# Picsart-AI-Research/MI-GAN

Hardware: AMD Instinct MI355X
Metric: images/sec migan-512 generator fwd (higher is better)
Workload: dtype f32; 1 GPU; migan-512 generator forward, batch=32 per GPU, 512x512, fp32 (BASELINE configs[2]); global_batch=32, resolution=512, parallelism=batch-shard x1, activation_storage=f32, streams=2, weights=static (migan_assume_static_weights: 1x1 operand planes prepared once)

## Files before the change

mi-gan_amd/csrc/migan_pipe.hpp:

```cpp
#pragma once

namespace migan {

constexpr int kPipeBWaves = 8;
constexpr int pipe_threads(int na) { return (na + kPipeBWaves) * 64; }

template <int MODE, int NT, int CIN, bool FROMRGB, int R>
struct PipeLds {
  static constexpr int NKC = CIN / 32;
  static constexpr int IN_SLOT = 1536 * 16;
  static constexpr int A_BUF = 2 * 128 * 64;
  static constexpr int B_CHUNK = 2 * NT * 64;
  static constexpr bool WRES = NKC * B_CHUNK <= 32 * 1024;
  static constexpr int NBUF_B = WRES ? NKC : 2;
  static constexpr int OFF_IN = 0;
  static constexpr int OFF_A = OFF_IN + R * IN_SLOT;
  static constexpr int OFF_B = OFF_A + 2 * A_BUF;
  static constexpr int OFF_W = OFF_B + NBUF_B * B_CHUNK;
  static constexpr bool TAPS_RES = NKC <= 8;
  static constexpr int OFF_F = OFF_W + (TAPS_RES ? NKC : 2) * 1280;
  static constexpr int F_SZ = FROMRGB ? NKC * 3 * 32 * 32 : 0;
  static constexpr int OFF_RGB = OFF_F + F_SZ;
  static constexpr int RGB_BUF = 192 * 32;
  static constexpr int OFF_T = OFF_RGB + (FROMRGB ? 2 * RGB_BUF : 0);
// ... 421 lines not shown
              const int hp = p.HO >> 1, wp = p.WO >> 1;
              const int row = lane / 10, col = lane - row * 10;
              const int yy = ((wtc.y * p.sy - p.off) >> 1) - 1 + row, xx = ((wtc.x * p.sx - p.off) >> 1) - 1 + col;
              const bool ok = lane < 60 && yy >= 0 && yy < hp && xx >= 0 && xx < wp;
              const unsigned voff = ok ? (unsigned)(yy * wp + xx) * 4u : 0xfffff000u;
              float* pw = reinterpret_cast<float*>(lds + L::OFF_PW + (wk & 1) * L::PW_SZ);
#pragma unroll
              for (int ch = 0; ch < 3; ++ch) MIGAN_LDS_DMA4(pbuf, voff, (unsigned)((wtc.b * 3 + ch) * hp * wp) * 4u, pw + ch * 64);
            }
            ++wk;
            if (wk < T) tile_next(wtc);
          }
          wstep = wstep + 1 == NKC ? 0 : wstep + 1;
        }
      };
      for (int g = 0; g < G; ++g) {
        if constexpr (!WRES) { if (g >= 1) issue_b(); }
        issue_prev_window();
        issue_in();
        if constexpr (!TAPS_RES) { if (g + 2 < G) load_taps((dc + 1) % NKC); }
        PPROF_MARK(0);
        if (g + 1 < G) depthwise(dslot, dc, (g + 1) & 1);
        PPROF_MARK(1);
        if constexpr (!TAPS_RES) { if (g + 2 < G) store_taps(g & 1); }
        dslot = dslot + 1 == R ? 0 : dslot + 1;
        dc = dc + 1 == NKC ? 0 : dc + 1;
        if (R == 3 && g + 3 < G) MIGAN_WAIT_VMCNT(DNI); else MIGAN_WAIT_VMCNT(0);
        PPROF_MARK(2);
        MIGAN_BARRIER_LDS();
        PPROF_MARK(3);
      }
    }
    if constexpr (TORGB) MIGAN_BARRIER_LDS();
    if constexpr (MODE == MODE_UP) {
#pragma unroll
      for (int i = 0; i < 2 * (NT / 64) - 1; ++i) MIGAN_BARRIER_LDS();
    }
    PPROF_END(AT);
    return;
  }

  const int tb = tid - AT, wb = wave_u - NA;
  const int rb = wb & 3, cbk = wb >> 2;
  const int l31 = lane & 31, half = lane >> 5;
  (void)tb;
  f16v acc[NTIW], accp[NTIW];
#pragma unroll
  for (int j = 0; j < NTIW; ++j)
#pragma unroll
    for (int r = 0; r < 16; ++r) { acc[j][r] = 0.0f; accp[j][r] = 0.0f; }

  auto mfma_chunk = [&](int abuf, int bbuf, bool first) {
    const char* ab = lds + L::OFF_A + abuf * L::A_BUF;
    const char* bb = lds + L::OFF_B + bbuf * L::B_CHUNK;
#pragma unroll
    for (int ks = 0; ks < KC / 16; ++ks) {
      f4 av[NPL], bv[NTIW][NPL];
      {
        const int row = rb * 32 + l31;
        const char* q = ab + row * PB + (((2 * ks + half) ^ ((row >> 2) & (NSLOT - 1))) << 4);
#pragma unroll
        for (int pl = 0; pl < NPL; ++pl) av[pl] = ld4(reinterpret_cast<const float*>(q + pl * MT * PB));
      }
#pragma unroll
      for (int j = 0; j < NTIW; ++j) {
        const int row = cbk * (NT / 2) + j * 32 + l31;
        const char* q = bb + row * PB + (((2 * ks + half) ^ ((row >> 2) & (NSLOT - 1))) << 4);
#pragma unroll
        for (int pl = 0; pl < NPL; ++pl) bv[j][pl] = ld4(reinterpret_cast<const float*>(q + pl * NT * PB));
      }
#pragma unroll
      for (int j = 0; j < NTIW; ++j) {
        if (first && ks == 0) acc[j] = f16v{0.f, 0.f, 0.f, 0.f, 0.f, 0.f, 0.f, 0.f, 0.f, 0.f, 0.f, 0.f, 0.f, 0.f, 0.f, 0.f};
        acc[j] = MIGAN_MFMA_F16_32X32X16(av[1], bv[j][0], acc[j]);
      }
#pragma unroll
      for (int j = 0; j < NTIW; ++j) acc[j] = MIGAN_MFMA_F16_32X32X16(av[0], bv[j][1], acc[j]);
#pragma unroll
      for (int j = 0; j < NTIW; ++j) acc[j] = MIGAN_MFMA_F16_32X32X16(av[0], bv[j][0], acc[j]);
    }
  };

  const float acc_scale = reinterpret_cast<const float*>(p.wsplit)[-4];
  const bool has_noise = p.noise != nullptr;
  const float ns = has_noise ? p.noise_strength[0] : 0.0f;
  const size_t img_out_bytes = (size_t)p.HO * p.WO * p.CO * 4;

  int ck = 0, cn0 = 0, cb0 = 0, cgy0 = 0, cgx0 = 0, pn0 = 0, pb0 = 0, pgy0 = 0, pgx0 = 0;
  int ppar = 0;
  TileCur ctc = tile0;
  tile_coords(ctc, cn0, cb0, cgy0, cgx0);
  auto hand_over = [&]() {
#pragma unroll
    for (int j = (MODE == MODE_NORMAL ? 1 : 0); j < NTIW; ++j) accp[j] = acc[j];
    pn0 = cn0; pb0 = cb0; pgy0 = cgy0; pgx0 = cgx0; ppar = ck & 1;
    if (++ck < T) { tile_next(ctc); tile_coords(ctc, cn0, cb0, cgy0, cgx0); }
  };

  BuildCursor bcur;
  if constexpr (FROMRGB) build_begin(bcur);
  auto build_step = [&](BuildCursor& bc) {
    build_units(bc, NA == 8 && wb >= 3 ? -1 : wb, 8);
    build_advance(bc);
  };
  MIGAN_BARRIER_LDS();
  if constexpr (FROMRGB) {
    build_step(bcur);
    build_step(bcur);
  }
  MIGAN_BARRIER_LDS();
  MIGAN_BARRIER_LDS();

  if constexpr (MODE == MODE_NORMAL) {
    float* const t_s = reinterpret_cast<float*>(lds + L::OFF_T) + wb * (32 * 32);
    const int q4 = lane & 7, prow = lane >> 3;
    int twr[4];
    {
      const int u = (l31 >> 2) ^ (2 * half);
#pragma unroll
      for (int v = 0; v < 4; ++v) twr[v] = (4 * half) * 32 + ((u ^ ((v & 1) + 4 * (v >> 1))) << 2) + (l31 & 3);
    }
    const int trd0 = prow * 32 + ((q4 ^ (prow >> 1)) << 2), trd1 = prow * 32 + ((q4 ^ (prow >> 1) ^ 4) << 2);
    float nz[4] = {0.f, 0.f, 0.f, 0.f};
    float nzn[4] = {0.f, 0.f, 0.f, 0.f};
    float rs[4][3];
    unsigned pix0 = 0;
    f4 tw[NTIW][3];
    float tbias[3] = {0.f, 0.f, 0.f};
    if constexpr (TORGB) {
#pragma unroll
      for (int ch = 0; ch < 3; ++ch) tbias[ch] = p.trgb_b[ch];
#pragma unroll
      for (int j = 0; j < NTIW; ++j)
#pragma unroll
        for (int ch = 0; ch < 3; ++ch) tw[j][ch] = ld4(p.trgb_w + ch * p.CO + cbk * (NT / 2) + j * 32 + q4 * 4);
    }
    float* const part_s = reinterpret_cast<float*>(lds + L::OFF_P) + rb * (32 * 4);
    u4v u8c = {0u, 0u, 0u, 0u}, u8n = {0u, 0u, 0u, 0u};
    auto request_next = [&]() {
      if (has_noise) {
        const unsigned px = (unsigned)((cgy0 + 2 * rb) * p.WO + cgx0 + prow) * 4u;
#pragma unroll
        for (int q = 0; q < 4; ++q) nzn[q] = *at_bytes(p.noise + ((q >> 1) * p.WO + (q & 1) * 8), px);
      }
      if constexpr (TORGB) {
        if (p.u8_out && cbk == 0 && q4 < 4)
          u8n = fetch_pixel_bytes(p.u8_img, p.u8_mask, (size_t)cb0 * p.HO * p.WO + (size_t)(cgy0 + 2 * rb + (q4 >> 1)) * p.WO + cgx0 + (q4 & 1) * 8 + prow);
      }
    };
    auto begin_tile_epilogue = [&]() {
      pix0 = (unsigned)((pgy0 + 2 * rb) * p.WO + pgx0 + prow);
#pragma unroll
      for (int q = 0; q < 4; ++q) nz[q] = nzn[q];
      if constexpr (TORGB) {
        u8c = u8n;
#pragma unroll
        for (int q = 0; q < 4; ++q) rs[q][0] = rs[q][1] = rs[q][2] = 0.0f;
      }
    };
    auto stage_block = [&](const f16v& a) {
      MIGAN_WAVE_SYNC();
#pragma unroll
      for (int r = 0; r < 16; ++r) t_s[twr[((r >> 1) & 1) + 2 * ((r >> 2) & 1)] + ((r & 3) + 8 * (r >> 2)) * 32] = a[r];
      MIGAN_WAVE_SYNC();
    };
    f4 tv[4];
    auto fetch_block = [&]() {
#pragma unroll
      for (int q = 0; q < 4; ++q) tv[q] = ld4(t_s + ((q & 1) ? trd1 : trd0) + q * 8 * 32);
    };
    const bool store_y = !TORGB || p.y != nullptr;
    auto finish_block = [&](int j) {
      char* yb = reinterpret_cast<char*>(p.y) + (size_t)pb0 * img_out_bytes;
      if constexpr (TORGB) {
        const unsigned col = (unsigned)(pn0 + cbk * (NT / 2) + j * 32 + q4 * 4);
        f4 v[4];
#pragma unroll
        for (int q = 0; q < 4; ++q) v[q] = act4(tv[q] * acc_scale + MIGAN_FMUL_RN(nz[q], ns));
        if (store_y) {
#pragma unroll
          for (int q = 0; q < 4; ++q) {
            const unsigned pix = pix0 + (unsigned)((q >> 1) * p.WO + (q & 1) * 8);
            Io<0>::st(yb, (pix * (unsigned)p.CO + col) * 4u, v[q]);
          }
        }
#pragma unroll
        for (int q = 0; q < 4; ++q) {
          float r0, r1, r2;
          torgb_partial(v[q], tw[j][0], tw[j][1], tw[j][2], r0, r1, r2);
          rs[q][0] += r0; rs[q][1] += r1; rs[q][2] += r2;
        }
      } else {
#pragma unroll
        for (int q = 0; q < 4; ++q) {
          f4 v = tv[q] * acc_scale + MIGAN_FMUL_RN(nz[q], ns);
          v = act4(v);
          const unsigned pix = pix0 + (unsigned)((q >> 1) * p.WO + (q & 1) * 8);
          Io<0>::st(yb, (pix * (unsigned)p.CO + (unsigned)(pn0 + cbk * (NT / 2) + j * 32 + q4 * 4)) * 4u, v);
        }
      }
    };
    float mine[3] = {0.f, 0.f, 0.f};
    auto rgb_partials = [&]() {
#pragma unroll
      for (int q = 0; q < 4; ++q) {
        const float s0 = MIGAN_SUM8(rs[q][0]), s1 = MIGAN_SUM8(rs[q][1]), s2 = MIGAN_SUM8(rs[q][2]);
        if (q4 == q) { mine[0] = s0; mine[1] = s1; mine[2] = s2; }
      }
      if (cbk == 1 && q4 < 4) st4(part_s + (8 * q4 + prow) * 4, f4{mine[0], mine[1], mine[2], 0.0f});
    };
    auto rgb_finish = [&]() {
      if (cbk == 0 && q4 < 4) {
        const f4 other = ld4(part_s + (8 * q4 + prow) * 4);
        const size_t plane = (size_t)p.HO * p.WO;
        const int oy = pgy0 + 2 * rb + (q4 >> 1), ox = pgx0 + (q4 & 1) * 8 + prow;
        float o3[3] = {mine[0] + other.x, mine[1] + other.y, mine[2] + other.z};
        MIGAN_OPAQUE_F(o3[0]); MIGAN_OPAQUE_F(o3[1]); MIGAN_OPAQUE_F(o3[2]);
        o3[0] += tbias[0]; MIGAN_OPAQUE_F(o3[0]);
        o3[1] += tbias[1]; MIGAN_OPAQUE_F(o3[1]);
        o3[2] += tbias[2]; MIGAN_OPAQUE_F(o3[2]);
        if (p.img_prev) {
          const int y0 = (oy & 1) ? (oy >> 1) : (oy >> 1) - 1, x0 = (ox & 1) ? (ox >> 1) : (ox >> 1) - 1;
          const float wy0 = (oy & 1) ? 0.75f : 0.25f, wx0 = (ox & 1) ? 0.75f : 0.25f;
          const float* pw = reinterpret_cast<const float*>(lds + L::OFF_PW + ppar * L::PW_SZ) + (y0 - (pgy0 >> 1) + 1) * 10 + (x0 - (pgx0 >> 1) + 1);
#pragma unroll
          for (int ch = 0; ch < 3; ++ch) {
            const float r0 = wx0 * pw[ch * 64] + (1.0f - wx0) * pw[ch * 64 + 1];
            const float r1 = wx0 * pw[ch * 64 + 10] + (1.0f - wx0) * pw[ch * 64 + 11];
            o3[ch] = (wy0 * r0 + (1.0f - wy0) * r1) + o3[ch];
          }
        }
        if (p.u8_out) {
          compose_pixel_bytes(u8c, p.u8_out, (size_t)pb0 * plane + (size_t)oy * p.WO + ox, o3[0], o3[1], o3[2]);
        } else {
          const unsigned po = (unsigned)(oy * p.WO + ox) * 4u;
#pragma unroll
          for (int ch = 0; ch < 3; ++ch) *at_bytes(p.img_out + ((size_t)pb0 * 3 + ch) * plane, po) = o3[ch];
        }
      }
    };
#pragma unroll
    for (int c = 0; c < NKC; ++c) {
      mfma_chunk(c & 1, WRES ? c : (c & 1), c == 0);
      if (c == NKC - 1) {
        request_next();
        stage_block(acc[0]);
        hand_over();
      }
      if constexpr (FROMRGB) build_step(bcur);
      MIGAN_BARRIER_LDS();
    }
    for (int t = 1; t < T; ++t) {
#pragma unroll
      for (int c = 0; c < NKC; ++c) {
        PPROF_MARK(7);
        if (c < NTIW) fetch_block();
        mfma_chunk(c & 1, WRES ? c : (c & 1), c == 0);
        PPROF_MARK(4);
        if (c == NKC - 1) request_next();
        PPROF_MARK(12);
        if (c == 0) begin_tile_epilogue();
        PPROF_MARK(5);
        if (c < NTIW) {
          finish_block(c);
          if (c + 1 < NTIW) stage_block(accp[c + 1 < NTIW ? c + 1 : 0]);
        }
        PPROF_MARK(9);
        if constexpr (TORGB) {
          if (c == NTIW - 1) rgb_partials();
          PPROF_MARK(10);
          if (c == NTIW) rgb_finish();
          PPROF_MARK(11);
        }
        if (c == NKC - 1) {
          stage_block(acc[0]);
          hand_over();
        }
        PPROF_MARK(7);
        if constexpr (FROMRGB) build_step(bcur);
        PPROF_MARK(13);
        MIGAN_BARRIER_LDS();
        PPROF_MARK(6);
      }
    }
    begin_tile_epilogue();
#pragma unroll
    for (int j = 0; j < NTIW; ++j) {
      fetch_block();
      finish_block(j);
      if (j + 1 < NTIW) stage_block(accp[j + 1 < NTIW ? j + 1 : 0]);
    }
    if constexpr (TORGB) {
      rgb_partials();
      MIGAN_BARRIER_LDS();
      rgb_finish();
    }
  } else {
    constexpr int GS = 64 + 4, QN = 16, LG_QN = 4, NH = NT / 64;
    static_assert(NT == 64 || NT == 128, "FIR-up tiles: 64 or 128 output channels");
    constexpr int SP = NKC / NH;
    static_assert(NKC % NH == 0 && SP >= 2, "too few K steps to hide the FIR epilogue under");
    constexpr int BT = kPipeBWaves * 64;
    constexpr int STEP = BT >> LG_QN;
    constexpr int ITEMS = MT * QN / BT;
    float* const g_s = reinterpret_cast<float*>(lds + L::OFF_T);
    auto acc_to_lds = [&](int h) {
      if (NH == 2 && cbk != h) return;
#pragma unroll
      for (int j = 0; j < NTIW; ++j)
#pragma unroll
        for (int r = 0; r < 16; ++r) {
          const int row = rb * 32 + (r & 3) + 8 * (r >> 2) + 4 * half;
          const int ly = pgy0 + (row >> lgGW), lx = pgx0 + (row & (GW - 1));
          float v = accp[j][r];
          if (ly < 0 || ly >= p.H || lx < 0 || lx >= p.W) v = 0.0f;
          g_s[row * GS + (NH == 2 ? j * 32 : cbk * 32) + l31] = v;
        }
    };
    const int c4 = tb & (QN - 1), m0 = tb >> LG_QN;
    struct ItemIo {
      f4 sk[2][2];
      float nzv[2][2];
    };
    auto item_geo = [&](int k, int h, int& m, unsigned& lpix, unsigned& loff) -> bool {
      m = m0 + k * STEP;
      const int gy = m >> lgGW, gx = m & (GW - 1);
      if (gy < 1 || gy > GH - 2 || gx < 1 || gx > GW - 2) return false;
      const int ly = pgy0 + gy, lx = pgx0 + gx;
      if (ly >= p.H || lx >= p.W) return false;
      lpix = (unsigned)((2 * ly) * p.WO + 2 * lx);
      loff = (lpix * (unsigned)p.CO + (unsigned)(pn0 + h * 64 + c4 * 4)) * 4u;
      return true;
    };
    auto item_load = [&](int k, int h, ItemIo& io) {
      int m;
      unsigned lpix, loff;
      if (!item_geo(k, h, m, lpix, loff)) return;
      const char* sb = p.skip ? reinterpret_cast<const char*>(p.skip) + (size_t)pb0 * img_out_bytes : nullptr;
#pragma unroll
      for (int a = 0; a < 2; ++a)
#pragma unroll
        for (int bb = 0; bb < 2; ++bb) {
          const unsigned dp = (unsigned)(a * p.WO + bb);
          io.nzv[a][bb] = has_noise ? p.noise[lpix + dp] : 0.0f;
          io.sk[a][bb] = sb ? Io<0>::ld_once(sb, loff + dp * (unsigned)p.CO * 4u) : f4{0.f, 0.f, 0.f, 0.f};
        }
    };
    auto item_finish = [&](int k, int h, const ItemIo& io) {
      int m;
      unsigned lpix, loff;
      if (!item_geo(k, h, m, lpix, loff)) return;
      char* yb = reinterpret_cast<char*>(p.y) + (size_t)pb0 * img_out_bytes;
      f4 e[3], o[3];
#pragma unroll
      for (int dy = 0; dy < 3; ++dy) {
        const float* gp = g_s + (m + (dy - 1) * GW) * GS + c4 * 4;
        const f4 l = ld4(gp - GS), ctr = ld4(gp), rgt = ld4(gp + GS);
        e[dy] = 0.25f * l + 0.75f * ctr;
        o[dy] = 0.75f * ctr + 0.25f * rgt;
      }
      f4 out[2][2];
      out[0][0] = 0.25f * e[0] + 0.75f * e[1];
      out[0][1] = 0.25f * o[0] + 0.75f * o[1];
      out[1][0] = 0.75f * e[1] + 0.25f * e[2];
      out[1][1] = 0.75f * o[1] + 0.25f * o[2];
#pragma unroll
      for (int a = 0; a < 2; ++a)
#pragma unroll
        for (int bb = 0; bb < 2; ++bb) {
          f4 v = out[a][bb] * acc_scale + MIGAN_FMUL_RN(io.nzv[a][bb], ns);
          v = act4(v);
          v += io.sk[a][bb];
          Io<0>::st(yb, loff + (unsigned)(a * p.WO + bb) * (unsigned)p.CO * 4u, v);
        }
    };
    constexpr int SL = SP - 1;
    auto slice_of = [](int k) { return k * SL / ITEMS; };
    ItemIo io[2];
#pragma unroll
    for (int c = 0; c < NKC; ++c) {
      mfma_chunk(c & 1, WRES ? c : (c & 1), c == 0);
      if (c == NKC - 1) hand_over();
      MIGAN_BARRIER_LDS();
    }
    for (int t = 1; t < T; ++t) {
#pragma unroll
      for (int c = 0; c < NKC; ++c) {
        constexpr int dummy = 0; (void)dummy;
        const int h = c / SP, cs = c % SP;
        if (cs >= 1) {
#pragma unroll
          for (int k = 0; k < ITEMS; ++k)
            if (slice_of(k) == cs - 1 && (k == 0 || slice_of(k - 1) != cs - 1)) item_load(k, h, io[k & 1]);
        }
        PPROF_MARK(7);
        mfma_chunk(c & 1, WRES ? c : (c & 1), c == 0);
        PPROF_MARK(4);
        if (cs == 0) {
          acc_to_lds(h);
        } else {
#pragma unroll
          for (int k = 0; k < ITEMS; ++k)
            if (slice_of(k) == cs - 1) {
              if (k + 1 < ITEMS && slice_of(k + 1) == cs - 1) item_load(k + 1, h, io[(k + 1) & 1]);
              item_finish(k, h, io[k & 1]);
            }
        }
        if (c == NKC - 1) hand_over();
        PPROF_MARK(5);
        MIGAN_BARRIER_LDS();
        PPROF_MARK(6);
      }
    }
#pragma unroll
    for (int h = 0; h < NH; ++h) {
      if (h > 0) MIGAN_BARRIER_LDS();
      acc_to_lds(h);
      MIGAN_BARRIER_LDS();
      item_load(0, h, io[0]);
#pragma unroll
      for (int k = 0; k < ITEMS; ++k) {
        if (k + 1 < ITEMS) item_load(k + 1, h, io[(k + 1) & 1]);
        item_finish(k, h, io[k & 1]);
      }
    }
  }
  PPROF_MARK(5);
  PPROF_END(AT);
}

template <int NT, int CIN, int R>
struct DownLds {
  static constexpr int KC = 16, NKC = CIN / KC;
  static constexpr int IN_UNITS = 12 * 36 * 4;
  static constexpr int A_BUF = 2 * 64 * 32;
  static constexpr int B_CHUNK = 2 * NT * 32;
  static constexpr bool WRES = NKC * B_CHUNK <= 32 * 1024;
  static constexpr int NBUF_B = WRES ? NKC : 2;
  static constexpr int DWP = 17;
  static constexpr int D_SZ = 10 * 2 * DWP * KC * 4;
  static constexpr int IN_SLOT = IN_UNITS * 16;
  static constexpr int OFF_D = R * IN_SLOT;
  static constexpr int OFF_A = OFF_D + D_SZ;
  static constexpr int OFF_B = OFF_A + 2 * A_BUF;
  static constexpr int OFF_W = OFF_B + NBUF_B * B_CHUNK;
  static constexpr int OFF_T = OFF_W + NKC * 640;
  template <int NB> static constexpr int total() { return OFF_T + NB * 32 * 32 * 4; }
};

template <int NT, int CIN, int R, int NA, int NB>
MIGAN_GLOBAL void MIGAN_LAUNCH_BOUNDS((NA + NB) * 64, (NA + NB) / 4) sepconv_pipedown_kernel(const SepArgs p) {
  typedef DownLds<NT, CIN, R> L;
  constexpr int AT = NA * 64, KC = 16, QC = 4, LG_QC = 2, NKC = L::NKC, MT = 64, GH = 4, GW = 16, lgGW = 4;
  constexpr int IGH = 12, IGW = 36, NPIXW = IGH * IGW, NITEMS = NPIXW * QC, DH = 10, DW = 34, DH2 = 5, DWP = L::DWP;
  constexpr int DNI = (NITEMS + AT - 1) / AT;
  constexpr bool WRES = L::WRES;
  constexpr int DNB = (4 * NT + AT - 1) / AT;
  static_assert(NB == 4 || NB == 8, "2 row blocks x 2 or 4 column groups");
  constexpr int NTIW = NT * 2 / (32 * NB);
  constexpr bool DEFER = NTIW <= 2;
  static_assert(NTIW <= NKC, "one epilogue block per K step");
  static_assert(NT == 128 || NT == 256, "one workgroup owns 128 or 256 output channels");
  static_assert(R == 2, "two-slot ring");
  static_assert(L::template total<NB>() <= 160 * 1024, "LDS budget");
  MIGAN_DYN_SMEM(smem);
  char* const lds = reinterpret_cast<char*>(smem);
  constexpr int IN_SLOT = L::IN_SLOT, OFF_D = L::OFF_D, OFF_A = L::OFF_A, OFF_B = L::OFF_B, OFF_W = L::OFF_W, OFF_T = L::OFF_T;

  const int tid = threadIdx.x;
  const int lane = tid & 63;
  const int wave_u = MIGAN_UNIFORM(tid >> 6);
  const bool groupA = tid < AT;
  const int HO = p.H >> 1, WO = p.W >> 1;

  const int ntiles = p.tiles_x * p.tiles_y * p.nchunks * p.B;
  const int xcd = (int)blockIdx.x & 7;
  const int tq = ntiles >> 3, tr = ntiles & 7;
  const int tcnt = tq + (xcd < tr ? 1 : 0);
  const int tbase = xcd < tr ? xcd * (tq + 1) : tr * (tq + 1) + (xcd - tr) * tq;
  const int tstep = ((int)gridDim.x + 7 - xcd) >> 3;
  const int tl0 = (int)blockIdx.x >> 3;
  const int T = tl0 < tcnt ? (tcnt - tl0 + tstep - 1) / tstep : 0;
  if (T == 0) return;
  const int G = T * NKC;
  PPROF_BEGIN();
  struct TileCur {
    int n, x, y, b;
  };
  const int st_n = tstep % p.nchunks, st_r1 = tstep / p.nchunks;
  const int st_x = st_r1 % p.tiles_x, st_r2 = st_r1 / p.tiles_x;
  const int st_y = st_r2 % p.tiles_y, st_b = st_r2 / p.tiles_y;
  TileCur tile0;
  {
    int t = tbase + tl0;
    tile0.n = t % p.nchunks; t /= p.nchunks;
    tile0.x = t % p.tiles_x; t /= p.tiles_x;
    tile0.y = t % p.tiles_y;
    tile0.b = t / p.tiles_y;
  }
  auto tile_next = [&](TileCur& c) {
    int carry = 0;
    c.n += st_n;
    if (c.n >= p.nchunks) { c.n -= p.nchunks; carry = 1; }
    c.x += st_x + carry; carry = 0;
    if (c.x >= p.tiles_x) { c.x -= p.tiles_x; carry = 1; }
    c.y += st_y + carry; carry = 0;
    if (c.y >= p.tiles_y) { c.y -= p.tiles_y; carry = 1; }
    c.b += st_b + carry;
  };

  if (groupA) {
    MIGAN_SETPRIO(2);
    const int lt = tid;
    float* const w_s = reinterpret_cast<float*>(lds + OFF_W);
    float* const d_s = reinterpret_cast<float*>(lds + OFF_D);
    for (int i = lt; i < CIN * 9 / 4; i += AT) {
      const f4 v = ld4(p.wdw + i * 4);
#pragma unroll
      for (int e = 0; e < 4; ++e) {
        const int f = i * 4 + e, ch = f / 9, tap = f - ch * 9;
        w_s[(ch >> 4) * 160 + tap * 16 + (ch & 15)] = v[e];
      }
    }
    for (int i = lt; i < CIN / 4; i += AT) st4(w_s + ((i * 4) >> 4) * 160 + 144 + ((i * 4) & 15), ld4(p.bdw + i * 4));

    const MIGAN_BUF wbuf = MIGAN_MAKE_BUF(p.wsplit, (unsigned)(2 * p.CO * CIN) * 2u);
    const bool bshort = MIGAN_UNIFORM((DNB - 1) * AT + wave_u * 64) >= 4 * NT;
    unsigned dboff[DNB];
#pragma unroll
    for (int j = 0; j < DNB; ++j) {
      const int u = lt + j * AT;
      const int plane = u / (2 * NT), rem = u % (2 * NT);
      dboff[j] = (unsigned)(plane * p.CO * CIN + (rem >> 1) * 32 + (rem & 1) * 8) * 2u;
    }
    auto dma_b = [&](int n0_, int chunk, int buf) {
      float* bb = reinterpret_cast<float*>(lds + OFF_B + buf * L::B_CHUNK);
      const unsigned soff = (unsigned)((chunk >> 1) * 32 * p.CO + n0_ * 32 + (chunk & 1) * 16) * 2u;
#pragma unroll
      for (int j = 0; j < DNB; ++j)
        if (j + 1 < DNB || !bshort) MIGAN_LDS_DMA16(wbuf, dboff[j], soff, bb + (j * AT + wave_u * 64) * 4);
    };
    const bool dshort = MIGAN_UNIFORM((DNI - 1) * AT + wave_u * 64) >= NITEMS;
    unsigned dgoff[DNI], drel[DNI], tile_soff = 0;
#pragma unroll
    for (int j = 0; j < DNI; ++j) {
      const int i = lt + j * AT;
      drel[j] = 0xfffff000u;
      if (i < NITEMS) {
        const int c4 = i & (QC - 1), pix = i >> LG_QC;
        drel[j] = (unsigned)(((pix / IGW) * p.W + (pix % IGW)) * CIN + c4 * 4) * 4u;
      }
    }
    auto make_dgoff = [&](int gy0_, int gx0_) {
      const int iy0 = 2 * gy0_ - 2, ix0 = 2 * gx0_ - 2;
      if (iy0 >= 0 && iy0 + IGH <= p.H && ix0 >= 0 && ix0 + IGW <= p.W) {
#pragma unroll
        for (int j = 0; j < DNI; ++j) dgoff[j] = drel[j];
        tile_soff = (unsigned)((iy0 * p.W + ix0) * CIN) * 4u;
        return;
      }
      tile_soff = 0;
#pragma unroll
      for (int j = 0; j < DNI; ++j) {
        const int i = lt + j * AT;
        unsigned g = 0xfffff000u;
        if (i < NITEMS) {
          const int c4 = i & (QC - 1), pix = i >> LG_QC;
          const int yy = iy0 + pix / IGW, xx = ix0 + pix % IGW;
          if (yy >= 0 && yy < p.H && xx >= 0 && xx < p.W) g = (unsigned)((yy * p.W + xx) * CIN + c4 * 4) * 4u;
        }
        dgoff[j] = g;
      }
    };
    const unsigned img_bytes = (unsigned)(p.H * p.W * CIN) * 4u;
    auto dma_in = [&](int b0_, int chunk, int slot) {
      float* in_s = reinterpret_cast<float*>(lds + slot * IN_SLOT);
      const MIGAN_BUF xbuf = MIGAN_MAKE_BUF(reinterpret_cast<const char*>(p.x) + (size_t)b0_ * img_bytes, img_bytes);
#pragma unroll
      for (int j = 0; j < DNI; ++j)
        if (j + 1 < DNI || !dshort) MIGAN_LDS_DMA16(xbuf, dgoff[j], tile_soff + (unsigned)(chunk * KC) * 4u, in_s + (j * AT + wave_u * 64) * 4);
    };
    auto stage1 = [&](int slot, int chunk, int gy0_, int gx0_) {
      const float* in_s = reinterpret_cast<const float*>(lds + slot * IN_SLOT);
      const float* wc = w_s + chunk * 160;
      const int c4 = lt & (QC - 1);
      f4 w[9];
#pragma unroll
      for (int tap = 0; tap < 9; ++tap) w[tap] = ld4(wc + tap * KC + c4 * 4);
      const f4 bias = ld4(wc + KC * 9 + c4 * 4);
      const int yim0 = 2 * gy0_ - 1, xim0 = 2 * gx0_ - 1;
      for (int it = lt; it < DH2 * DW * QC; it += AT) {
        const int r = it >> LG_QC;
        const int dx = r % DW, dy0 = 2 * (r / DW);
        const float* ip = in_s + (dy0 * IGW + dx) * KC + c4 * 4;
        f4 win[4][3];
#pragma unroll
        for (int rr = 0; rr < 4; ++rr) {
          win[rr][0] = ld4(ip); win[rr][1] = ld4(ip + KC); win[rr][2] = ld4(ip + 2 * KC);
          ip += IGW * KC;
        }
        const int xim = xim0 + dx;
        const bool colin = xim >= 0 && xim < p.W;
        float* dp = d_s + ((dy0 * 2 + (dx & 1)) * DWP + (dx >> 1)) * KC + c4 * 4;
        f4 dv[2];
#pragma unroll
        for (int o = 0; o < 2; ++o) {
          f4 sacc = bias;
#pragma unroll
          for (int ky = 0; ky < 3; ++ky)
#pragma unroll
            for (int kx = 0; kx < 3; ++kx) sacc += w[ky * 3 + kx] * win[o + ky][kx];
          const int yim = yim0 + dy0 + o;
          dv[o] = f4{0.f, 0.f, 0.f, 0.f};
          if (colin && yim >= 0 && yim < p.H) dv[o] = act4(sacc);
        }
        st4(dp, 0.125f * dv[0] + 0.375f * dv[1]);
        st4(dp + 2 * DWP * KC, 0.375f * dv[0] + 0.125f * dv[1]);
      }
    };
    auto stage2 = [&](int abuf) {
      char* a_b = lds + OFF_A + abuf * L::A_BUF;
      for (int it = lt; it < MT * QC; it += AT) {
        const int c4 = it & (QC - 1), m = it >> LG_QC;
        const int ox = m & (GW - 1), oy = m >> lgGW;
        const float* dp = d_s + ((2 * oy) * 2 * DWP + ox) * KC + c4 * 4;
        f4 a = {0.f, 0.f, 0.f, 0.f};
#pragma unroll
        for (int kx = 0; kx < 4; ++kx) {
          const float fx = (kx == 0 || kx == 3) ? 0.125f : 0.375f;
          const float* q = dp + ((kx & 1) * DWP + (kx >> 1)) * KC;
          a += fx * (ld4(q) + ld4(q + 3 * 2 * DWP * KC));
        }
        u2v h1, h2;
        split2_f16(a * kF16AScale, h1, h2);
        char* d = a_b + m * 32 + c4 * 8;
        *reinterpret_cast<u2v*>(d) = h1;
        *reinterpret_cast<u2v*>(d + MT * 32) = h2;
      }
    };

    int is = 0, ic = 0, ik = 0, ib0 = 0, in0 = 0, igy0 = 0, igx0 = 0;
    TileCur itc = tile0;
    auto icoords = [&]() { in0 = itc.n * NT; ib0 = itc.b; igy0 = itc.y * GH; igx0 = itc.x * GW; };
    icoords();
    make_dgoff(igy0, igx0);
    auto issue = [&]() {
      if (is < G) {
        dma_in(ib0, ic, is & 1);
        ++is;
        if (++ic == NKC) {
          ic = 0;
          if (++ik < T) { tile_next(itc); icoords(); make_dgoff(igy0, igx0); }
        }
      }
    };
    int bs = 0, bc = 0, bk = 0, bn0 = in0;
    TileCur btc = tile0;
    auto issue_b = [&]() -> bool {
      if (bs >= G) return false;
      dma_b(bn0, bc, bs & 1);
      ++bs;
      if (++bc == NKC) {
        bc = 0;
        if (++bk < T) { tile_next(btc); bn0 = btc.n * NT; }
      }
      return true;
    };
    int dk = 0, dc = 0, dgy0 = igy0, dgx0 = igx0;
    TileCur dtc = tile0;
    auto dadvance = [&]() {
      if (++dc == NKC) {
        dc = 0;
        if (++dk < T) { tile_next(dtc); dgy0 = dtc.y * GH; dgx0 = dtc.x * GW; }
      }
    };
    if constexpr (WRES) {
#pragma unroll
      for (int c = 0; c < NKC; ++c) dma_b(in0, c, c);
    } else {
      issue_b();
      issue_b();
    }
    issue();
    issue();
    if (dshort) MIGAN_WAIT_VMCNT(DNI - 1); else MIGAN_WAIT_VMCNT(DNI);
    MIGAN_BARRIER_LDS();
    stage1(0, 0, dgy0, dgx0);
    MIGAN_BARRIER_LDS();
    stage2(0);
    dadvance();
    MIGAN_WAIT_VMCNT(0);
    MIGAN_BARRIER_LDS();
    for (int g = 0; g < G; ++g) {
      issue();
      PPROF_MARK(0);
      if (g + 1 < G) stage1((g + 1) & 1, dc, dgy0, dgx0);
      PPROF_MARK(1);
      MIGAN_BARRIER_LDS();
      PPROF_MARK(3);
      if (g + 1 < G) { stage2((g + 1) & 1); dadvance(); }
      PPROF_MARK(14);
      bool newer = false;
      if constexpr (!WRES) newer = issue_b();
      if (newer && !bshort) MIGAN_WAIT_VMCNT(DNB); else if (newer && DNB > 1) MIGAN_WAIT_VMCNT(DNB > 1 ? DNB - 1 : 0); else MIGAN_WAIT_VMCNT(0);
      PPROF_MARK(2);
      MIGAN_BARRIER_LDS();
      PPROF_MARK(3);
    }
    PPROF_END(AT);
    return;
  }

  const int wb = wave_u - NA;
  const int rb = wb & 1, cb = wb >> 1;
  const int l31 = lane & 31, half = lane >> 5;
  f16v acc[NTIW], accp[DEFER ? NTIW : 1];
#pragma unroll
  for (int j = 0; j < NTIW; ++j)
#pragma unroll
    for (int r = 0; r < 16; ++r) { acc[j][r] = 0.0f; if (DEFER) accp[j][r] = 0.0f; }
  auto mfma_chunk = [&](int abuf, int bbuf, bool first) {
    const char* ab = lds + OFF_A + abuf * L::A_BUF + (rb * 32 + l31) * 32 + half * 16;
    const char* bb = lds + OFF_B + bbuf * L::B_CHUNK + half * 16;
    const f4 a_hi = ld4(reinterpret_cast<const float*>(ab)), a_lo = ld4(reinterpret_cast<const float*>(ab + MT * 32));
    f4 b_hi[NTIW], b_lo[NTIW];
#pragma unroll
    for (int j = 0; j < NTIW; ++j) {
      const char* q = bb + ((cb * NTIW + j) * 32 + l31) * 32;
// ... 125 lines not shown
```

Measured before the change: 3662 images/sec.

## Compact FIR-up epilogue item map to interior pixels and hand-schedule item loads

The FIR-up epilogue used to map work items over the whole halo tile and discard border ones with branches. It now maps items only over interior pixels, clamping coordinates so every lane does useful work, and replaces the general slice schedule with a fixed three-item schedule. Noise and skip loads become branch-free masked loads from a dummy pointer, and the first item's loads are issued during hand-over to hide latency. The static_asserts tie the code to a single 64-column phase with exactly three items, so other tile shapes will no longer compile.

```diff
diff --git a/mi-gan_amd/csrc/migan_pipe.hpp b/mi-gan_amd/csrc/migan_pipe.hpp
--- a/mi-gan_amd/csrc/migan_pipe.hpp
+++ b/mi-gan_amd/csrc/migan_pipe.hpp
@@ -747,7 +747,12 @@
     static_assert(NKC % NH == 0 && SP >= 2, "too few K steps to hide the FIR epilogue under");
     constexpr int BT = kPipeBWaves * 64;
     constexpr int STEP = BT >> LG_QN;
-    constexpr int ITEMS = MT * QN / BT;
+    constexpr int IH = GH - 2, IW = GW - 2;
+    constexpr int NIT = IH * IW * QN;
+    constexpr int FULL = NIT / BT, ITEMS = (NIT + BT - 1) / BT;
+    constexpr int RWAVES = (NIT - FULL * BT) / 64;
+    static_assert((NIT - FULL * BT) % 64 == 0, "the remainder of the item map must be whole waves");
+    static_assert(NH == 1 && FULL == 2 && ITEMS == 3 && SP - 1 == ITEMS, "item schedule: one 64-column phase, items 0 and 1 for all, item 2 for RWAVES waves");
     float* const g_s = reinterpret_cast<float*>(lds + L::OFF_T);
     auto acc_to_lds = [&](int h) {
       if (NH == 2 && cbk != h) return;
@@ -763,38 +768,41 @@
         }
     };
     const int c4 = tb & (QN - 1), m0 = tb >> LG_QN;
+    const bool third = wb < RWAVES;
+    const bool has_skip = p.skip != nullptr;
     struct ItemIo {
       f4 sk[2][2];
       float nzv[2][2];
     };
-    auto item_geo = [&](int k, int h, int& m, unsigned& lpix, unsigned& loff) -> bool {
-      m = m0 + k * STEP;
-      const int gy = m >> lgGW, gx = m & (GW - 1);
-      if (gy < 1 || gy > GH - 2 || gx < 1 || gx > GW - 2) return false;
-      const int ly = pgy0 + gy, lx = pgx0 + gx;
-      if (ly >= p.H || lx >= p.W) return false;
-      lpix = (unsigned)((2 * ly) * p.WO + 2 * lx);
+    auto item_geo = [&](int k, int h, int& m, unsigned& lpix, unsigned& loff) {
+      const int q = m0 + k * STEP;
+      const int ty = 1 + q / IW, tx = 1 + q % IW, ylast = p.H - 1 - pgy0, xlast = p.W - 1 - pgx0;
+      const int gy = ty < ylast ? ty : ylast, gx = tx < xlast ? tx : xlast;
+      m = (gy << lgGW) + gx;
+      lpix = (unsigned)((2 * (pgy0 + gy)) * p.WO + 2 * (pgx0 + gx));
       loff = (lpix * (unsigned)p.CO + (unsigned)(pn0 + h * 64 + c4 * 4)) * 4u;
-      return true;
-    };
-    auto item_load = [&](int k, int h, ItemIo& io) {
+    };
+    auto item_load = [&](int k, int h, ItemIo& io, bool live) {
       int m;
       unsigned lpix, loff;
-      if (!item_geo(k, h, m, lpix, loff)) return;
-      const char* sb = p.skip ? reinterpret_cast<const char*>(p.skip) + (size_t)pb0 * img_out_bytes : nullptr;
+      item_geo(k, h, m, lpix, loff);
+      const bool ln = has_noise && live, ls = has_skip && live;
+      const float* nb = ln ? p.noise : reinterpret_cast<const float*>(p.wsplit);
+      const char* sb = ls ? reinterpret_cast<const char*>(p.skip) + (size_t)pb0 * img_out_bytes : reinterpret_cast<const char*>(p.wsplit);
+      const unsigned nmask = ln ? ~0u : 0u, smask = ls ? ~0u : 0u;
 #pragma unroll
       for (int a = 0; a < 2; ++a)
 #pragma unroll
         for (int bb = 0; bb < 2; ++bb) {
           const unsigned dp = (unsigned)(a * p.WO + bb);
-          io.nzv[a][bb] = has_noise ? p.noise[lpix + dp] : 0.0f;
-          io.sk[a][bb] = sb ? Io<0>::ld_once(sb, loff + dp * (unsigned)p.CO * 4u) : f4{0.f, 0.f, 0.f, 0.f};
+          io.nzv[a][bb] = nb[(lpix + dp) & nmask];
+          io.sk[a][bb] = Io<0>::ld_once(sb, (loff + dp * (unsigned)p.CO * 4u) & smask);
         }
     };
     auto item_finish = [&](int k, int h, const ItemIo& io) {
       int m;
       unsigned lpix, loff;
-      if (!item_geo(k, h, m, lpix, loff)) return;
+      item_geo(k, h, m, lpix, loff);
       char* yb = reinterpret_cast<char*>(p.y) + (size_t)pb0 * img_out_bytes;
       f4 e[3], o[3];
 #pragma unroll
@@ -813,62 +821,56 @@
       for (int a = 0; a < 2; ++a)
 #pragma unroll
         for (int bb = 0; bb < 2; ++bb) {
-          f4 v = out[a][bb] * acc_scale + MIGAN_FMUL_RN(io.nzv[a][bb], ns);
+          const float nz = has_noise ? io.nzv[a][bb] : 0.0f;
+          f4 v = out[a][bb] * acc_scale + MIGAN_FMUL_RN(nz, ns);
           v = act4(v);
-          v += io.sk[a][bb];
+          v += has_skip ? io.sk[a][bb] : f4{0.f, 0.f, 0.f, 0.f};
           Io<0>::st(yb, loff + (unsigned)(a * p.WO + bb) * (unsigned)p.CO * 4u, v);
         }
     };
-    constexpr int SL = SP - 1;
-    auto slice_of = [](int k) { return k * SL / ITEMS; };
     ItemIo io[2];
 #pragma unroll
     for (int c = 0; c < NKC; ++c) {
       mfma_chunk(c & 1, WRES ? c : (c & 1), c == 0);
-      if (c == NKC - 1) hand_over();
+      if (c == NKC - 1) {
+        hand_over();
+        item_load(0, 0, io[0], true);
+      }
       MIGAN_BARRIER_LDS();
     }
     for (int t = 1; t < T; ++t) {
 #pragma unroll
       for (int c = 0; c < NKC; ++c) {
-        constexpr int dummy = 0; (void)dummy;
-        const int h = c / SP, cs = c % SP;
-        if (cs >= 1) {
-#pragma unroll
-          for (int k = 0; k < ITEMS; ++k)
-            if (slice_of(k) == cs - 1 && (k == 0 || slice_of(k - 1) != cs - 1)) item_load(k, h, io[k & 1]);
-        }
         PPROF_MARK(7);
         mfma_chunk(c & 1, WRES ? c : (c & 1), c == 0);
         PPROF_MARK(4);
-        if (cs == 0) {
-          acc_to_lds(h);
+        if (c == 0) {
+          acc_to_lds(0);
+        } else if (c == 1) {
+          item_load(1, 0, io[1], true);
+          item_finish(0, 0, io[0]);
+        } else if (c == 2) {
+          item_load(2, 0, io[0], third);
+          item_finish(1, 0, io[1]);
         } else {
-#pragma unroll
-          for (int k = 0; k < ITEMS; ++k)
-            if (slice_of(k) == cs - 1) {
-              if (k + 1 < ITEMS && slice_of(k + 1) == cs - 1) item_load(k + 1, h, io[(k + 1) & 1]);
-              item_finish(k, h, io[k & 1]);
-            }
-        }
-        if (c == NKC - 1) hand_over();
+          if (third) item_finish(2, 0, io[0]);
+        }
+        if (c == NKC - 1) {
+          hand_over();
+          item_load(0, 0, io[0], true);
+        }
         PPROF_MARK(5);
         MIGAN_BARRIER_LDS();
         PPROF_MARK(6);
       }
     }
-#pragma unroll
-    for (int h = 0; h < NH; ++h) {
-      if (h > 0) MIGAN_BARRIER_LDS();
-      acc_to_lds(h);
-      MIGAN_BARRIER_LDS();
-      item_load(0, h, io[0]);
-#pragma unroll
-      for (int k = 0; k < ITEMS; ++k) {
-        if (k + 1 < ITEMS) item_load(k + 1, h, io[(k + 1) & 1]);
-        item_finish(k, h, io[k & 1]);
-      }
-    }
+    acc_to_lds(0);
+    MIGAN_BARRIER_LDS();
+    item_load(1, 0, io[1], true);
+    item_finish(0, 0, io[0]);
+    item_load(2, 0, io[0], third);
+    item_finish(1, 0, io[1]);
+    if (third) item_finish(2, 0, io[0]);
   }
   PPROF_MARK(5);
   PPROF_END(AT);
```

Result: no change. 3683 images/sec, median of 6 (+0.6%).
